# CUAI/Edge-Proposal-Sets

Measured on AMD Instinct MI355X. Metric: candidate edges scored/sec on ogbl-ppa (ppa-like synthetic): Adamic-Adar over the FULL 2-hop non-edge candidate set + top-4M selection, higher is better.
Workload: dtype int64

## Files before the change

### edge-proposal-sets_amd/_lib.py

```python
from __future__ import annotations

import ctypes
import os
import subprocess
import threading

_HERE = os.path.dirname(os.path.abspath(__file__))
LIB_PATH = os.path.join(_HERE, "libeps_hip.so")
CSRC = os.path.join(_HERE, "csrc")

_c = ctypes
_vp, _i64, _i32, _int = _c.c_void_p, _c.c_int64, _c.c_int32, _c.c_int

SIGNATURES = {
    "eps_version": (_int, []),
    "eps_last_error": (_c.c_char_p, []),
    "eps_device_info": (_int, [_c.POINTER(_int), _c.c_char_p, _int]),
    "eps_warm_up": (_int, []),
    "eps_col_sums": (_int, [_vp, _vp, _vp, _i64, _i64, _vp, _vp, _vp]),
    "eps_node_weights": (_int, [_vp, _i64, _int, _vp, _vp]),
    "eps_node_weights_f64": (_int, [_vp, _i64, _int, _vp, _vp]),
    "eps_pair_scores": (_int, [_vp, _vp, _vp, _vp, _i64, _vp, _vp, _i64, _vp, _vp, _vp, _vp]),
    "eps_pair_scores_f64": (_int, [_vp, _vp, _vp, _vp, _i64, _vp, _vp, _i64, _vp, _vp, _vp]),
    "eps_pair_scores_grouped": (_int, [_vp, _vp, _vp, _vp, _i64, _vp, _vp, _i64, _vp, _vp, _vp, _vp]),
# ... 60 lines not shown
    "eps_mlp_decode_bn_stats": (_int, [_vp, _i64, _i32, _vp, _vp, _i64, _c.POINTER(_vp), _c.POINTER(_vp), _i32, _vp, _vp, _vp, _i64, _vp]),
    "eps_mlp_decode_bn_backward": (_int, [_vp, _i64, _i32, _vp, _vp, _i64, _c.POINTER(_vp), _c.POINTER(_vp), _c.POINTER(_vp), _i32,
                                          _c.POINTER(_vp), _c.POINTER(_vp), _vp, _vp, _vp, _c.c_float, _vp, _c.c_float, _vp, _vp, _vp,
                                          _c.POINTER(_vp), _c.POINTER(_vp), _vp, _vp, _vp, _vp, _i64, _vp]),
    "eps_kth_largest_workspace_bytes": (_i64, []),
    "eps_kth_largest_f32": (_int, [_vp, _i64, _i64, _vp, _vp, _vp]),
    "eps_select_topk_rows_relabelled": (_int, [_vp, _vp, _i64, _i64, _i32, _vp, _vp, _vp, _vp, _i64, _vp]),
    "eps_select_topk_rows_pairs": (_int, [_vp, _vp, _i64, _i64, _i32, _vp, _vp, _i64, _vp, _vp, _i64, _vp]),
    "eps_sort_pairs_by_u_workspace_bytes": (_i64, [_i64]),
    "eps_sort_pairs_by_u": (_int, [_vp, _i64, _i32, _i32, _vp, _vp, _i64, _vp]),
    "eps_compact_between": (_int, [_vp, _vp, _i64, _vp, _vp, _vp, _vp, _vp, _vp]),
    "eps_select_compact_workspace_bytes": (_i64, []),
    "eps_select_compact": (_int, [_vp, _vp, _i64, _vp, _i64, _i32, _c.c_float, _c.c_float, _c.c_float, _vp, _vp, _vp, _vp, _i64, _vp, _vp, _vp]),
    "eps_kth_begin": (_int, [_vp, _i64, _vp]),
    "eps_kth_hist_f32": (_int, [_vp, _i64, _vp, _i32, _vp]),
    "eps_kth_pick": (_int, [_vp, _i32, _vp, _vp]),
    "eps_compact_at_least": (_int, [_vp, _vp, _i64, _vp, _vp, _vp, _vp, _vp]),
    "eps_select_topk_cut_workspace_bytes": (_i64, []),
    "eps_compact_survivors": (_int, [_vp, _vp, _i64, _vp, _vp, _vp, _vp, _i64, _vp]),
    "eps_select_topk_cut": (_int, [_vp, _vp, _i64, _i64, _vp, _vp, _vp, _vp, _i64, _vp]),
    "eps_select_topk_rows_workspace_bytes": (_i64, [_i64]),
    "eps_select_topk_rows": (_int, [_vp, _vp, _i64, _i64, _i32, _vp, _vp, _vp, _i64, _vp]),
    "eps_tail_state_bytes": (_i64, []),
    "eps_score_bins": (_i32, []),
    "eps_score_hist_into": (_int, [_vp, _vp, _i64, _vp, _vp, _vp, _vp, _vp]),
    "eps_score_deal_plan": (_int, [_vp, _i64, _i32, _i64, _vp, _vp, _vp, _vp, _vp, _vp]),
    "eps_score_hist": (_int, [_vp, _vp, _i64, _vp, _vp, _vp, _vp, _vp]),
    "eps_score_pick_compact": (_int, [_vp, _vp, _i64, _vp, _vp, _vp, _i64, _i32, _c.c_float, _c.c_float, _c.c_float, _i32, _vp, _vp, _vp,
                                      _vp, _i64, _vp, _vp, _vp]),
    "eps_radix_sort_workspace_bytes": (_i64, [_i64]),
    "eps_radix_sort_by_u": (_int, [_vp, _i64, _vp, _i32, _i32, _vp, _vp, _i64, _vp, _vp]),
    "eps_radix_sort_rows": (_int, [_vp, _vp, _i64, _vp, _i64, _i32, _vp, _vp, _i64, _vp, _vp, _vp, _i64, _vp, _vp]),
    "eps_rescore_runs_dev": (_int, [_vp, _vp, _vp, _i64, _vp, _i64, _vp, _vp, _vp]),
    "eps_pack_keys": (_int, [_vp, _vp, _i64, _i64, _vp, _vp]),
    "eps_unpack_keys": (_int, [_vp, _i64, _vp, _vp, _vp]),
    "eps_two_path_counts": (_int, [_vp, _vp, _i64, _vp, _vp]),
    "eps_katz_workspace_bytes": (_i64, [_i64]),
    "eps_katz_pair_scores": (_int, [_vp, _vp, _vp, _vp, _vp, _vp, _vp, _vp, _i64, _vp, _vp, _i64, _c.c_double, _c.c_double,
                                    _c.c_double, _vp, _vp, _vp]),
    "eps_katz_columns_limits": (_int, [_c.POINTER(_i32), _c.POINTER(_i32)]),
    "eps_katz_columns_workspace_bytes": (_i64, [_i64]),
    "eps_katz_columns_chunk": (_i64, [_i64]),
    "eps_katz_column_scores": (_int, [_vp, _vp, _vp, _vp, _vp, _vp, _vp, _i64, _i64, _i64, _vp, _vp, _i64, _c.c_double, _c.c_double,
                                      _c.c_double, _i64, _i32, _vp, _i64, _vp, _vp]),
    "eps_cos_node_features": (_int, [_vp, _vp, _vp, _i64, _vp, _i64, _i32, _vp, _i64, _vp]),
    "eps_edge_cosines": (_int, [_vp, _vp, _i64, _vp, _i64, _i32, _vp, _vp, _vp]),
    "eps_cos_node_features_nrm": (_int, [_vp, _vp, _vp, _i64, _vp, _i64, _i32, _vp, _i64, _vp, _vp]),
    "eps_pair_cn_backward_workspace_bytes": (_i64, [_i64]),
    "eps_pair_cn_backward": (_int, [_vp, _vp, _vp, _i64, _i64, _vp, _vp, _vp, _i64, _vp, _vp, _i64, _vp]),
    "eps_cos_features_backward": (_int, [_vp, _vp, _vp, _i64, _vp, _i64, _i32, _vp, _vp, _vp, _vp, _vp, _i64, _vp]),
    "eps_csr_merge_workspace_bytes": (_i64, [_i64]),
    "eps_csr_merge_count": (_int, [_vp, _vp, _i64, _vp, _i64, _vp, _vp, _vp, _vp, _i64, _vp]),
    "eps_csr_merge_fill": (_int, [_vp, _vp, _vp, _i64, _vp, _i64, _vp, _vp, _i64, _vp, _vp, _vp]),
    "eps_segment_topk_class_max": (_i64, [_i32]),
    "eps_segment_topk": (_int, [_vp, _vp, _vp, _i64, _i64, _vp, _vp, _vp, _vp]),
    "eps_local_index_pairs": (_int, [_vp, _i64, _vp, _vp, _vp, _i64, _i32, _vp, _vp]),
    "eps_local_index_columns_workspace_bytes": (_i64, [_i64]),
    "eps_local_index_columns": (_int, [_vp, _i64, _i64, _i64, _vp, _vp, _vp, _i64, _vp, _vp, _i32, _vp, _vp, _i64, _vp, _vp, _vp, _vp,
                                       _i64, _vp]),
    "eps_pair_cn_list_limits": (_int, [_c.POINTER(_i32), _c.POINTER(_i32)]),
    "eps_pair_cn_list_count": (_int, [_vp, _vp, _i64, _vp, _vp, _i64, _vp, _vp]),
    "eps_pair_cn_list_fill": (_int, [_vp, _vp, _i64, _vp, _vp, _i64, _vp, _vp, _vp, _vp]),
    "eps_cn_list_transpose_workspace_bytes": (_i64, [_i64, _i64]),
    "eps_cn_list_transpose": (_int, [_vp, _vp, _i64, _i64, _i64, _vp, _vp, _vp, _i64, _vp]),
    "eps_local_community_limits": (_int, [_c.POINTER(_i32), _c.POINTER(_i32), _c.POINTER(_i32)]),
    "eps_local_community_degrees": (_int, [_vp, _vp, _i64, _vp, _vp, _i64, _vp, _vp, _vp]),
# ... 92 lines not shown
```

### edge-proposal-sets_amd/csrc/eps_common.hip

```cpp
#include "eps_common.h"

#include <stdarg.h>
#include <string.h>

#include <atomic>

static thread_local char g_err[512] = "";

void eps_set_error(const char *fmt, ...)
{
    va_list ap;
    va_start(ap, fmt);
    vsnprintf(g_err, sizeof(g_err), fmt, ap);
    va_end(ap);
}

extern "C" const char *eps_last_error(void) { return g_err; }

extern "C" int eps_version(void) { return EPS_ABI_VERSION; }

int eps_num_cus()
{
    static thread_local int cached_dev = -1;
    static thread_local int cached_cus = 256;
// ... 35 lines not shown
    if (hipGetSymbolAddress((void **)counter, HIP_SYMBOL(g_work_counter)) != hipSuccess) {
        eps_set_error("%s: cannot resolve the work counter", who);
        return EPS_ELAUNCH;
    }
    *counter += g_counter_turn.fetch_add(1) % EPS_COUNTER_SLOTS;
    if (hipMemsetAsync(*counter, 0, sizeof(unsigned int), stream) != hipSuccess) {
        eps_set_error("%s: cannot reset the work counter", who);
        return EPS_ELAUNCH;
    }
    return EPS_OK;
}

__device__ unsigned int g_work_counter8[EPS_COUNTER_SLOTS][8];
static std::atomic<unsigned int> g_counter8_turn{0};

int eps_take_counters8(unsigned int **counters, hipStream_t stream, const char *who)
{
    if (hipGetSymbolAddress((void **)counters, HIP_SYMBOL(g_work_counter8)) != hipSuccess) {
        eps_set_error("%s: cannot resolve the work counters", who);
        return EPS_ELAUNCH;
    }
    *counters += 8 * (g_counter8_turn.fetch_add(1) % EPS_COUNTER_SLOTS);
    if (hipMemsetAsync(*counters, 0, 8 * sizeof(unsigned int), stream) != hipSuccess) {
        eps_set_error("%s: cannot reset the work counters", who);
        return EPS_ELAUNCH;
    }
    return EPS_OK;
}

#define EPS_UNITS(X) \
    X(graph_prep) X(csr_merge) X(scan_pieces) X(scan_tables) X(scan_heads) X(rescore) \
    X(pair_intersect) X(pair_grouped) X(expand_score) X(filter_scan) X(spmm_csr) \
    X(gemm_f32) X(dense_cn) X(mlp_decode) X(mlp_decode_bf16) X(mlp_decode_train) X(topk_keys) X(topk_select) X(segment_topk) \
    X(tail_sort) X(katz_pairs) X(katz_columns) X(local_index) X(cosine_cn) X(cosine_cn_bwd) X(pair_cn_list) X(local_community)

#define EPS_DECLARE_WARM(unit) extern "C" void eps_warm_##unit(void *stream);
EPS_UNITS(EPS_DECLARE_WARM)

extern "C" int eps_warm_up(void)
{
    hipStream_t s = nullptr;
    if (hipStreamCreateWithFlags(&s, hipStreamNonBlocking) != hipSuccess) {
        eps_set_error("eps_warm_up: cannot create a stream");
        return EPS_ELAUNCH;
    }
#define EPS_CALL_WARM(unit) eps_warm_##unit(s);
    EPS_UNITS(EPS_CALL_WARM)
    const hipError_t e = hipStreamSynchronize(s);
    (void)hipStreamDestroy(s);
    if (e != hipSuccess) {
        eps_set_error("eps_warm_up: %s", hipGetErrorString(e));
        return EPS_ELAUNCH;
    }
    return EPS_OK;
}
```

### edge-proposal-sets_amd/csrc/tail_sort.hip

```cpp
#include "eps_common.h"
#include <string.h>

#define TS_T 1024
#define TS_W (TS_T / 64)
#define TS_KPT 4
#define TS_TILE (TS_T * TS_KPT)
#define TS_MAXG 256
#define TS_MAXPASS 16

#define TS_MB 8
#define TS_BINS ((32 - TS_MB + 1) << TS_MB)

__device__ __forceinline__ uint32_t ts_ordered(float f)
{
    f = f + 0.0f;
    const uint32_t b = __builtin_bit_cast(uint32_t, f);
    return (b & 0x80000000u) ? ~b : (b | 0x80000000u);
}
__device__ __forceinline__ float ts_unordered(uint32_t o)
{
    const uint32_t b = (o & 0x80000000u) ? (o & 0x7fffffffu) : ~o;
    return __builtin_bit_cast(float, b);
}
__device__ __forceinline__ uint32_t ts_bucket(uint32_t d)
{
    if (d < (1u << TS_MB)) return d;
    const int e = 31 - __clz((int)d);
    return ((uint32_t)(e - TS_MB + 1) << TS_MB) | ((d >> (e - TS_MB)) & ((1u << TS_MB) - 1u));
}
__device__ __forceinline__ uint32_t ts_bucket_floor(uint32_t b)
{
    if (b < (1u << TS_MB)) return b;
    const uint32_t e1 = b >> TS_MB, m = b & ((1u << TS_MB) - 1u);
    return ((1u << TS_MB) | m) << (e1 - 1u);
}

struct ts_sel_state {
    uint32_t hist[TS_BINS];
    uint32_t done;
    uint32_t pad;
    unsigned long long n_out;
};

struct ts_sort_state {
    uint32_t arrive;
    uint32_t leave;
    unsigned long long runs;
    uint32_t totals[TS_MAXPASS][256];
    uint32_t hist[TS_MAXG][256];
};

extern "C" int64_t eps_tail_state_bytes(void)
{
    const size_t a = (sizeof(ts_sel_state) + 255) & ~(size_t)255, b = (sizeof(ts_sort_state) + 255) & ~(size_t)255;
    return (int64_t)(a + b);
}
static ts_sel_state *ts_sel_of(void *state) { return (ts_sel_state *)state; }
static ts_sort_state *ts_sort_of(void *state) { return (ts_sort_state *)((char *)state + ((sizeof(ts_sel_state) + 255) & ~(size_t)255)); }

__global__ __launch_bounds__(TS_T) void ts_hist_kernel(const int64_t *__restrict__ keys, const float *__restrict__ vals, int64_t n_max,
                                                       const unsigned long long *__restrict__ n_dev, const float *__restrict__ base,
                                                       const float *__restrict__ above, uint32_t *__restrict__ hist)
{
    __shared__ uint32_t h[TS_BINS];
    const int tid = threadIdx.x, lane = tid & 63;
    int64_t n = n_max;
    if (n_dev) {
        const unsigned long long c = *n_dev;
// ... 741 lines not shown
```

### edge-proposal-sets_amd/ops.py

```python
from __future__ import annotations

import ctypes
import struct
from typing import Optional, Sequence, Tuple

import torch

from . import _lib

W_AA, W_RA = 0, 1

KERNEL_EVENTS = None
EVENT_NAMES = None
_SCAN_EVENTS = ("scan_piece_kernel", "filter_scan_kernel")

_SCRATCH = {}


def _scratch(name, dev, n_words: int, alloc, zero: bool = False) -> torch.Tensor:
    key = (name, dev.type, dev.index)
    buf = _SCRATCH.get(key)
    if buf is None or buf.numel() < n_words:
        _SCRATCH.pop(key, None)
        buf = None
# ... 1548 lines not shown
        _call("eps_sort_pairs_by_u", dev, keys, n, int(id_bits), int(v_block_shift), out, wsp, wsb, timed=("sort_pairs_by_u", n))
    return out


def _topk_rows(sel_keys, sel_vals, m: int, k: int, id_bits: int, perm, as_pairs: bool = False):
    dev = _need_gpu(sel_keys, sel_vals, perm)
    _chk(_I64, sel_keys=sel_keys, perm=perm); _chk(_F32, sel_vals=sel_vals)
    k = int(k)
    take = min(k, 2 * m)
    rows = torch.empty((2, take) if as_pairs else take, dtype=_I64, device=dev)
    out_v = torch.empty(take, dtype=_F32, device=dev)
    if take:
        _, wsp, wsb = _aligned_ws(dev, _lib.load().eps_select_topk_rows_workspace_bytes(m))
        head = (sel_keys, sel_vals, m, k, int(id_bits))
        if as_pairs:
            _call("eps_select_topk_rows_pairs", dev, *head, perm, rows, take, out_v, wsp, wsb, timed=("select_rows", m))
        elif perm is None:
            _call("eps_select_topk_rows", dev, *head, rows, out_v, wsp, wsb)
        else:
            _call("eps_select_topk_rows_relabelled", dev, *head, perm, rows, out_v, wsp, wsb)
    return rows, out_v


def select_rows(sel_keys: torch.Tensor, sel_vals: torch.Tensor, k: int, id_bits: int = 32,
                perm: Optional[torch.Tensor] = None) -> Tuple[torch.Tensor, torch.Tensor]:
    return _topk_rows(sel_keys, sel_vals, sel_keys.numel(), k, id_bits, perm)


def select_rows_pairs(sel_keys: torch.Tensor, sel_vals: torch.Tensor, k: int, id_bits: int = 32,
                      perm: Optional[torch.Tensor] = None) -> Tuple[torch.Tensor, torch.Tensor]:
    return _topk_rows(sel_keys, sel_vals, sel_keys.numel(), k, id_bits, perm, as_pairs=True)


def select_topk(keys: torch.Tensor, vals: torch.Tensor, k: int, id_bits: int = 32) -> Tuple[torch.Tensor, torch.Tensor]:
    dev = _need_gpu(keys, vals)
    _chk(_I64, keys=keys); _chk(_F32, vals=vals)
    n, k = keys.numel(), int(k)
    if vals.numel() != n:
        raise _lib.EpsError("select_topk: keys and vals differ in length")
    sel_k = torch.empty(n, dtype=_I64, device=dev)
    sel_v = torch.empty(n, dtype=_F32, device=dev)
    n_sel = torch.zeros(1, dtype=_I64, device=dev)
    _, wsp, wsb = _aligned_ws(dev, _lib.load().eps_select_topk_cut_workspace_bytes())
    _call("eps_select_topk_cut", dev, keys, vals, n, k, sel_k, sel_v, n_sel, wsp, wsb)
    return _topk_rows(sel_k, sel_v, int(n_sel.item()), k, id_bits, None)


def tail_state(dev) -> torch.Tensor:
    return _scratch(("tail", torch.cuda.current_stream(dev).cuda_stream), dev, 1,
                    lambda: (int(_lib.load().eps_tail_state_bytes()) + 7) // 8 + 32, zero=True)


def _tail_addr(dev):
    st = tail_state(dev)
    return ctypes.c_void_p(st.data_ptr() + (-st.data_ptr()) % 256)


def tail_state_reset(dev) -> None:
    tail_state(dev).zero_()


def score_hist(keys: Optional[torch.Tensor], vals: torch.Tensor, n_dev, base: torch.Tensor, above: Optional[torch.Tensor] = None) -> None:
    dev = _need_gpu(keys, vals, base, above)
    _chk(_I64, keys=keys, n_dev=n_dev); _chk(_F32, vals=vals, base=base, above=above)
    _call("eps_score_hist", dev, keys, vals, vals.numel(), n_dev, base, above, _tail_addr(dev),
          timed=("select_compact", vals.numel()))
# ... 109 lines not shown
```

### edge-proposal-sets_amd/scan.py

```python
from __future__ import annotations

from collections import namedtuple
from typing import List, Optional, Tuple

import torch

from . import ops
from .graph import CSRGraph

SAMPLE_STRIDE = 256
SAFETY = 2.0
SMALL_SET = 1 << 25
MAX_K = 1 << 30
MAX_LAUNCHES = 8
_CHUNK_SLACK = 8192 * 320
RELABEL_MIN_NODES = 100_000
ONE_PASS = True
_PIECE_SLACK = 8192 * 1024 + 65536
MAX_SCREEN_SHIFT = 30
HEADS = True
HEAD_BETA = 0.5
HEAD_KEEP = (0.3, 0.58)
HEAD_LIST = 2
HEAD_MIN_PATHS = 1 << 30
# ... 578 lines not shown
        bar = torch.where(torch.isinf(vote), -inf, vote)
    return bar


def _gather_varlen(t: torch.Tensor, world: int):
    from . import dist as epd
    n = torch.tensor([t.numel()], dtype=torch.int64, device=t.device)
    lens = torch.cat(epd.all_gather_list(n)).tolist()
    return epd.gather_ragged(t, lens)


def select_topk(keys: torch.Tensor, vals: torch.Tensor, k: int, n_nodes: Optional[int] = None) -> Tuple[torch.Tensor, torch.Tensor]:
    if keys.is_cuda:
        bits = 32 if not n_nodes else max(1, min(32, int(n_nodes - 1).bit_length()))
        return ops.select_topk(keys.contiguous(), vals.contiguous(), k, bits)
    return select_topk_torch(keys, vals, k)


def select_topk_torch(keys: torch.Tensor, vals: torch.Tensor, k: int) -> Tuple[torch.Tensor, torch.Tensor]:
    k2 = (k + 1) // 2
    if vals.numel() > k2:
        kth = torch.sort(vals, descending=True).values[k2 - 1] if k2 >= 1 else float("inf")
        m = vals >= kth
        keys, vals = keys[m], vals[m]
    keys = torch.cat([keys, ((keys & 0xFFFFFFFF) << 32) | (keys >> 32)])
    vals = torch.cat([vals, vals])
    o = torch.argsort(keys)
    keys, vals = keys[o], vals[o]
    o = torch.sort(vals, descending=True, stable=True).indices[:k]
    return keys[o], vals[o]


TAIL_DEVICE = True
TAIL_SORT = "library"
EXACT_SCREENING = True
RESCORE_V_BLOCK = 12
DIST_HIST = True
DIST_ROWS_MIN = 1 << 15


def score_splitters(vals: torch.Tensor, world: int) -> torch.Tensor:
    n = vals.numel()
    samp = torch.sort(vals[::max(1, n // 32768)], descending=True).values
    idx = (torch.arange(1, world, device=vals.device) * samp.numel()) // world
    return samp[idx.clamp(max=samp.numel() - 1)]


def score_range_counts(vals: torch.Tensor, splitters: torch.Tensor) -> torch.Tensor:
    r = (vals.unsqueeze(1) < splitters.unsqueeze(0)).sum(1)
    return torch.bincount(r, minlength=splitters.numel() + 1)


def _ordered_rows_distributed(keys: torch.Tensor, vals: torch.Tensor, k: int, bits: int, perm, rank: int, world: int,
                              rows_on: Optional[int] = None):
    from . import dist as epd
    sp = score_splitters(vals, world)
    counts = score_range_counts(vals, sp).tolist()
    lo = sp[rank:rank + 1] if rank < world - 1 else None
    hi = sp[rank - 1:rank] if rank > 0 else None
    mk, mv, _ = ops.compact_between(keys, vals, lo, hi)
    m = counts[rank]
    rk, rv = ops.select_rows(mk[:m].contiguous(), mv[:m].contiguous(), 2 * m, bits, perm)
    lens = [2 * c for c in counts]
    if rows_on is None:
        rows_k, rows_v = epd.gather_ragged(rk, lens), epd.gather_ragged(rv, lens)
    else:
        rows_k, rows_v = epd.gather_ragged_to(rk, lens, rows_on), epd.gather_ragged_to(rv, lens, rows_on)
# ... 129 lines not shown
                action = "heads off" if head_trouble >= 2 or head_stale >= 3 else "grow walked list" if overflow else "rebuild heads"
                return again(action, "launches with skipped heads", drop_heads)
        slot_overflow = any(t.slots > capacity for t in table)
        if screened and not self.rescore_all and not slot_overflow and any(table[0].cut < t.pre_thr for t in table):
            return again("rescore all", "the re-scoring pre-filter", drop_heads)
        if slot_overflow:
            return Verdict("rescan wider" if table[0].cut_is_neg_inf else "rescan below cut", launches, drop_heads, head_trouble, head_stale)
        n_cand, n_sel = sum(t.candidates for t in table), sum(t.n_sel for t in table)
        if bar_set and n_sel < (k2 if head_budget is not None else min(k2, n_cand)):
            return Verdict("drop bar" if launches > 3 else "lower bar", launches, drop_heads, head_trouble, head_stale)
        return Verdict("done", launches, drop_heads, head_trouble, head_stale)

    def apply(self, v: Verdict, total_half: int, world: int) -> str:
        self.launches, self.head_trouble, self.head_stale = v.launches, v.head_trouble, v.head_stale
        if v.action == "sketch off":
            self.sketch, self.sketch_void = False, self.sketch_void + 1
        elif v.action == "grow walked list":
            self.head_list *= 2
        elif v.action == "heads off":
            self.use_heads = False
        elif v.action == "rescore all":
            self.rescore_all = True
        elif v.action in ("rescan below cut", "rescan wider"):
            self.wanted *= 4
        elif v.action in ("lower bar", "drop bar"):
            self.safety = SAFETY * 8 ** (self.launches - 1)
            self.launches += 1
            if v.action == "drop bar":
                self.wanted = 2 * total_half // world
        return {"rescan below cut": "below cut", "lower bar": "estimate", "drop bar": "none"}.get(v.action, "keep")


def _device_tail(g: CSRGraph, screen: Screen, res: ops.Survivors, bar: torch.Tensor, k: int, k2: int, params, bits: int, perm):
    library = TAIL_SORT == "library"
    room = min(res.capacity, 2 * k2 + (1 << 16))
    while True:
        ops.score_hist(res.key, res.val, res.count_ptr, bar)
        c_keys, c_vals, n_valid, _, pre_thr = ops.score_pick_compact(res.key, res.val, res.count_ptr, bar, k2, mode=2,
                                                                     params=params, room=room, want_vals=screen.exact)
        count, sel_room = n_valid, room
        if library:
            nv = int(n_valid.item())
            if nv > room:
                room = min(res.capacity, nv)
                continue
            c_keys, c_vals = c_keys[:nv], c_vals[:nv] if screen.exact else None
            count, sel_room = None, max(nv, 1)
        if screen.exact:
            x_keys, x_vals = c_keys, c_vals
        elif library:
            x_keys = ops.sort_pairs_by_u(c_keys, bits, RESCORE_V_BLOCK)
            x_vals = ops.rescore_runs(g.rowptr, g.col, screen.fixw, g.n_rows, x_keys)
        else:
            x_keys = ops.radix_sort_by_u(c_keys, n_valid, bits, RESCORE_V_BLOCK)
            x_vals = ops.rescore_runs_dev(g.rowptr, g.col, screen.fixw, g.n_rows, x_keys, n_valid)
        ops.score_hist(x_keys, x_vals, count, bar, above=bar)
        sel_k, sel_v, n_sel, cut, _ = ops.score_pick_compact(x_keys, x_vals, count, bar, k2, above=bar, swap_halves=not screen.exact,
                                                             room=sel_room)
        row = (res.rec[1:2], res.rec[4:5], n_sel, cut, res.status, pre_thr, res.walked_slots, bar)
        if library:
            return [_unpack_status(_pack_status(*row).tolist())], sel_k, sel_v, cut, 0 if screen.exact else nv, None
        r_pairs, r_scores, n_rows = ops.radix_sort_rows(sel_k, sel_v, n_sel, k, bits, perm)
        st, (nv, n_out) = _unpack_status(_pack_status(*row, extra=(n_valid, n_rows)).tolist(), extra=2)
        if nv <= room:
            return [st], sel_k, sel_v, cut, 0 if screen.exact else nv, (r_pairs, r_scores, n_out)
        room = min(res.capacity, nv)


def _prefilter(g: CSRGraph, screen: Screen, res: ops.Survivors, bar, k2: int, params, world: int, rescore_all: bool):
    k_pre = 0 if rescore_all else (k2 + world - 1) // world
    room = res.capacity if rescore_all else min(res.capacity, 2 * k_pre + (1 << 16))
    c_keys, c_vals, n_valid, _, pre_thr = ops.select_compact(res.key, res.val, k_pre, res.count_ptr, mode=2, params=params, room=room)
    nv = int(n_valid.item())
    if nv > room:
        c_keys, c_vals, n_valid, _, pre_thr = ops.select_compact(res.key, res.val, k_pre, res.count_ptr, mode=2, params=params,
                                                                 room=min(res.capacity, nv))
        nv = int(n_valid.item())
    if screen.exact:
        return c_keys[:nv], c_vals[:nv], pre_thr, 0, room
    keys, vals = rescore_exact(g, screen, c_keys[:nv], bar)
    return keys, vals, pre_thr, nv, room


def _read_exchange(got: torch.Tensor, nsel_all: torch.Tensor, cut: torch.Tensor, counts: torch.Tensor, world: int):
    rows = got[:, :_STATUS_WORDS].reshape(-1).to(torch.int64)
    flat = torch.cat([rows, cut.view(torch.int32).to(torch.int64), nsel_all, counts.reshape(-1)]).tolist()
    nsel, deal = flat[rows.numel() + 1:][:world], flat[rows.numel() + 1 + world:]
    return ([_unpack_status(flat[r * _STATUS_WORDS:(r + 1) * _STATUS_WORDS])._replace(n_sel=nsel[r], cut_bits=flat[rows.numel()])
             for r in range(world)], [deal[r * world:(r + 1) * world] for r in range(world)])


def _cut_from_histograms(keys: torch.Tensor, vals: torch.Tensor, row, k2: int, bar: torch.Tensor, world: int):
    from . import dist as epd
    bins = ops.score_bins()
    send = torch.zeros(_XCHG_HEAD + bins, dtype=torch.int32, device=vals.device)
    send[:_STATUS_WORDS] = _pack_status(**row)
    ops.score_hist_into(keys, vals, None, bar, send[_XCHG_HEAD:], above=bar)
    got = epd._gather_into(send, world).view(world, _XCHG_HEAD + bins)
# ... 97 lines not shown
    g, perm = scan_graph(g0, relabel)
    fixw = _scan_weights(g0, g, perm, node_w) if g.val is None else None
    mine = shard_columns(g, rank, world)
    total_half = total_half_paths(g)
    k2 = (k + 1) // 2
    bits = max(1, min(32, int(g.n_rows - 1).bit_length()))
    screen = screen_weights(g0, g, perm, node_w) if one_pass_available(g) else None
    if screen is not None and not screen.usable:
        screen = None
    if screen is None and g.val is not None:
        raise ops._lib.EpsError("scan_topk: this weighted graph / weight table does not fit the one-pass scan (see scan_available)")
    slack = _CHUNK_SLACK if screen is None else _PIECE_SLACK
    sampled = total_half > SMALL_SET and SAFETY * k < total_half
    bar = estimate_bar(g, fixw, k, rank=rank, world=world, screen=screen) if sampled else None
    state = _Retry(int(sampled), (2 * total_half if bar is None else int(2 * SAFETY * k)) // world, HEAD_LIST, sketch=SKETCH_PIECES,
                   use_heads=bool(HEADS and screen is not None and screen.has_plan and screen.ssum is not None and g.val is None
                                  and total_half >= HEAD_MIN_PATHS))
    capacity = _capacity(state.wanted, slack)
    _count_scan(g, screen)
    n_rescored = None
    while True:
        if state.launches >= MAX_LAUNCHES:
            raise ops._lib.EpsError(f"scan_topk: no usable bar after {state.launches} launches (k = {k}, capacity {capacity})")
        def sketch_for(budget):
            return bool(state.sketch and screen is not None and screen_variant(g) == 2 and not screen.exact
                        and (int(screen.w_max_units) + 2) * SKETCH_PIECE_PATHS < 1 << 32
                        and budget >= HEAD_BETA * SKETCH_MIN_PATHS * screen.w_max_units)
        ht = (_heads_for(g, screen, bar, sketch_for) if state.use_heads and bar is not None else None)
        walked_cap = max(1, min(int(state.head_list * capacity), ops.SURVIVOR_SLOTS_MAX)) if ht is not None else 0
        res = _launch(g, fixw, mine if ht is None else live_columns(g, screen, ht, rank, world), float("-inf") if bar is None else bar,
                      capacity, both=True, screen=screen, heads=ht, walked_capacity=walked_cap, sketch=ht is not None and sketch_for(ht.budget))
        state.launches += 1
        rows = deal = None
        if screen is not None:
            params = screen.lower_params(max_degree(g), None if ht is None else ht.d_used) + (4e-6,)
        if (TAIL_DEVICE and not _sharded(world) and screen is not None and g.val is None and bar is not None and not state.rescore_all
                and k2 + (1 << 16) < (1 << 30)):
            table, sel_k, sel_v, cut, n_rescored, rows = _device_tail(g, screen, res, bar, k, k2, params, bits, perm)
        else:
            keys, vals, pre_thr, room = res.key, res.val, None, 0
            if screen is not None:
                keys, vals, pre_thr, n_rescored, room = _prefilter(g, screen, res, bar, k2, params, world, state.rescore_all)
            row = dict(slots=res.rec[1:2], candidates=res.rec[4:5], status=None if screen is None else res.status, pre_thr=pre_thr,
                       walked=res.walked_slots, bar=bar)
            exchange = _sharded(world) and screen is not None and not state.rescore_all
            sel_k, sel_v, cut, table, deal = (_cut_from_histograms(keys, vals, row, k2, bar, world) if exchange and bar is not None and DIST_HIST
                                              else _cut_from_scores(keys, vals, row, k2, room, world) if exchange
                                              else _cut_local(keys, vals, row, k2, screen is not None, world))
        v = state.verdict(table, capacity=capacity, walked_cap=walked_cap, head_budget=None if ht is None else ht.budget,
                          shift=None if ht is None else screen.shift, screened=screen is not None, k2=k2, bar_set=bar is not None)
        new_bar = state.apply(v, total_half, world)
        if v.drop_heads:
            screen.head_cur = None
        if v.action == "done":
            break
        if new_bar == "below cut":
            bar = torch.nextafter(cut, torch.full_like(cut, float("-inf")))
        elif new_bar == "estimate":
            bar = estimate_bar(g, fixw, k, safety=state.safety, rank=rank, world=world, screen=screen)
            if bar is None:
                state.wanted = 2 * total_half // world
        elif new_bar == "none":
            bar = None
        capacity = _capacity(state.wanted, slack)
    if screen is not None and bar is not None and 0.0 < table[0].bar < float("inf"):
        screen.bar_hint[(k, sample_stride(k), float(SAFETY))] = table[0].bar
    pairs, scores, shard = ((rows[0][:, :rows[2]], rows[1][:rows[2]], None) if rows is not None else
                            _ordered_rows(sel_k, sel_v, [t.n_sel for t in table], deal, k, bits, perm, rank, world, rows_on))
    if stats is not None:
        _step_stats(stats, g, screen, fixw, table, ht, capacity, state, n_rescored, shard, bar, rank, world)
    return pairs, scores
```

### include/eps_abi.h

```cpp
#ifndef EPS_ABI_H
#define EPS_ABI_H

#include <stdint.h>

#ifdef __cplusplus
extern "C" {
#endif

#define EPS_ABI_VERSION 7

#define EPS_OK 0
#define EPS_EINVAL (-1)
#define EPS_ELAUNCH (-2)
#define EPS_ENODEV (-3)

#define EPS_W_AA 0
#define EPS_W_RA 1

int eps_version(void);
const char *eps_last_error(void);

int eps_warm_up(void);

int eps_device_info(int *n_cu, char *name, int name_len);
// ... 224 lines not shown
int64_t eps_sort_pairs_by_u_workspace_bytes(int64_t n);
int eps_sort_pairs_by_u(const int64_t *keys, int64_t n, int32_t id_bits, int32_t v_block_shift, int64_t *out_by_u, void *workspace,
                        int64_t workspace_bytes, void *stream);
int64_t eps_select_topk_cut_workspace_bytes(void);
int eps_compact_survivors(const int64_t *keys, const float *vals, int64_t n, int64_t *out_keys, float *out_vals,
                          int64_t *n_out, void *workspace, int64_t workspace_bytes, void *stream);
int eps_compact_at_least(const int64_t *keys, const float *vals, int64_t n, const float *cut_or_null, int64_t *out_keys,
                         float *out_vals, int64_t *n_out, void *stream);
int eps_select_topk_cut(const int64_t *keys, const float *vals, int64_t n, int64_t k, int64_t *sel_keys, float *sel_vals,
                        int64_t *n_sel, void *workspace, int64_t workspace_bytes, void *stream);
int64_t eps_select_topk_rows_workspace_bytes(int64_t m);
int eps_select_topk_rows(const int64_t *sel_keys, const float *sel_vals, int64_t m, int64_t k, int32_t id_bits,
                         int64_t *out_keys, float *out_vals, void *workspace, int64_t workspace_bytes, void *stream);
int64_t eps_tail_state_bytes(void);
int32_t eps_score_bins(void);
int eps_score_hist_into(const int64_t *keys_or_null, const float *vals, int64_t n_max, const unsigned long long *n_dev_or_null,
                        const float *base, const float *above_or_null, uint32_t *hist, void *stream);
int eps_score_deal_plan(const uint32_t *hists, int64_t row_stride, int32_t world, int64_t k, const float *base, float *cut,
                        float *splitters, int64_t *counts, int64_t *nsel, void *stream);
int eps_score_hist(const int64_t *keys_or_null, const float *vals, int64_t n_max, const unsigned long long *n_dev_or_null,
                   const float *base, const float *above_or_null, void *state, void *stream);
int eps_score_pick_compact(const int64_t *keys_or_null, const float *vals, int64_t n_max, const unsigned long long *n_dev_or_null,
                           const float *base, const float *above_or_null, int64_t k, int32_t mode, float pa, float pb, float pc,
                           int32_t swap_halves, float *kth_or_null, float *thr_or_null, int64_t *out_keys_or_null,
                           float *out_vals_or_null, int64_t out_cap, int64_t *n_out_or_null, void *state, void *stream);
int64_t eps_radix_sort_workspace_bytes(int64_t n_records);
int eps_radix_sort_by_u(const int64_t *keys, int64_t n_max, const int64_t *n_dev_or_null, int32_t id_bits, int32_t v_block_shift,
                        int64_t *out_by_u, void *workspace, int64_t workspace_bytes, void *state, void *stream);
int eps_radix_sort_rows(const int64_t *sel_keys, const float *sel_vals, int64_t m_max, const int64_t *m_dev_or_null, int64_t k,
                        int32_t id_bits, const int64_t *perm_or_null, int64_t *out_pairs, int64_t out_ld, float *out_scores,
                        int64_t *n_rows_out_or_null, void *workspace, int64_t workspace_bytes, void *state, void *stream);
int eps_rescore_runs_dev(const int64_t *rowptr, const int32_t *col, const int64_t *fixw, int64_t n_nodes, const int64_t *keys,
                         int64_t n_max, const int64_t *n_dev, float *out, void *stream);
int eps_pack_keys(const float *score, const int64_t *ids_or_null, int64_t id_base, int64_t n,
                  int64_t *keys, void *stream);
int eps_unpack_keys(const int64_t *keys, int64_t n, float *score_or_null, int64_t *id_or_null,
                    void *stream);

int eps_two_path_counts(const int64_t *rowptr, const int32_t *col, int64_t n_nodes, int64_t *paths, void *stream);
int64_t eps_katz_workspace_bytes(int64_t n_pairs);
int eps_katz_pair_scores(const int64_t *rowptr, const int32_t *col, const float *val, const int64_t *rowptr_t,
                         const int32_t *col_t, const float *val_t, const int64_t *paths_out, const int64_t *paths_in,
                         int64_t n_nodes, const int32_t *u, const int32_t *v, int64_t n_pairs, double c1, double c2,
                         double c3, void *workspace, float *out, void *stream);

int eps_katz_columns_limits(int32_t *lds_capacity, int32_t *chunk);
int64_t eps_katz_columns_chunk(int64_t n_cand);
int64_t eps_katz_columns_workspace_bytes(int64_t max_support);
int eps_katz_column_scores(const int64_t *rowptr, const int32_t *col, const float *val, const int64_t *rowptr_t,
                           const int32_t *col_t, const float *val_t, const int64_t *paths_in, int64_t n_nodes,
                           int64_t v_lo, int64_t v_hi, const int64_t *colptr, const int32_t *cand_u, int64_t n_cand,
                           double c1, double c2, double c3, int64_t max_support, int32_t chunk, void *workspace,
                           int64_t workspace_bytes, float *out, void *stream);

int eps_cos_node_features(const int64_t *rowptr, const int32_t *col, const float *val, int64_t n_rows,
                          const float *x, int64_t ldx, int32_t f, float *xhat, int64_t ldh, void *stream);
int eps_edge_cosines(const int64_t *rowptr, const int32_t *col, int64_t n_rows, const float *xhat, int64_t ldh,
                     int32_t f, const int32_t *revpos, float *c, void *stream);

int eps_cos_node_features_nrm(const int64_t *rowptr, const int32_t *col, const float *val, int64_t n_rows,
                              const float *x, int64_t ldx, int32_t f, float *xhat, int64_t ldh, float *nrm, void *stream);
int64_t eps_pair_cn_backward_workspace_bytes(int64_t nnz);
int eps_pair_cn_backward(const int64_t *rowptr, const int32_t *col, const float *c, int64_t n_rows, int64_t nnz,
                         const int32_t *u, const int32_t *v, const float *g, int64_t n_pairs, float *gc, void *workspace,
                         int64_t workspace_bytes, void *stream);
int eps_cos_features_backward(const int64_t *rowptr, const int32_t *col, const float *val, int64_t n_rows,
// ... 44 lines not shown
```

Measured before the change: 1321 billion.

## Build top-k output rows by sorting all rescored pairs by score in one pass

Adds a device tail path that radix-sorts all rescored pairs by score in descending order, with swapped-halves keys as the tie-break. One block then finds the live count and the bucketed cut, and a windowed expand kernel writes both directed rows of each pair in rank order, resolving ties within equal-score runs. The default tail mode becomes this path whenever screening is inexact. It replaces the histogram, pick-compact and separate row-sort sequence with one full sort of n records, which may cost more than the old path when n is much larger than k2. If a tie run exceeds the window, the kernel sets a flag and the output falls back to the library path.

```diff
diff --git a/edge-proposal-sets_amd/_lib.py b/edge-proposal-sets_amd/_lib.py
--- a/edge-proposal-sets_amd/_lib.py
+++ b/edge-proposal-sets_amd/_lib.py
@@ -116,6 +116,10 @@
     "eps_radix_sort_by_u": (_int, [_vp, _i64, _vp, _i32, _i32, _vp, _vp, _i64, _vp, _vp]),
     "eps_radix_sort_rows": (_int, [_vp, _vp, _i64, _vp, _i64, _i32, _vp, _vp, _i64, _vp, _vp, _vp, _i64, _vp, _vp]),
     "eps_rescore_runs_dev": (_int, [_vp, _vp, _vp, _i64, _vp, _i64, _vp, _vp, _vp]),
+    "eps_rows_by_score_max_run": (_i32, []),
+    "eps_rows_by_score_window": (_i32, []),
+    "eps_rows_by_score_workspace_bytes": (_i64, [_i64]),
+    "eps_rows_by_score": (_int, [_vp, _vp, _i64, _vp, _i64, _i64, _i32, _vp, _vp, _vp, _vp, _vp, _vp, _vp, _i64, _vp, _vp, _i64, _vp]),
     "eps_pack_keys": (_int, [_vp, _vp, _i64, _i64, _vp, _vp]),
     "eps_unpack_keys": (_int, [_vp, _i64, _vp, _vp, _vp]),
     "eps_two_path_counts": (_int, [_vp, _vp, _i64, _vp, _vp]),
diff --git a/edge-proposal-sets_amd/csrc/eps_common.hip b/edge-proposal-sets_amd/csrc/eps_common.hip
--- a/edge-proposal-sets_amd/csrc/eps_common.hip
+++ b/edge-proposal-sets_amd/csrc/eps_common.hip
@@ -91,7 +91,7 @@
     X(graph_prep) X(csr_merge) X(scan_pieces) X(scan_tables) X(scan_heads) X(rescore) \
     X(pair_intersect) X(pair_grouped) X(expand_score) X(filter_scan) X(spmm_csr) \
     X(gemm_f32) X(dense_cn) X(mlp_decode) X(mlp_decode_bf16) X(mlp_decode_train) X(topk_keys) X(topk_select) X(segment_topk) \
-    X(tail_sort) X(katz_pairs) X(katz_columns) X(local_index) X(cosine_cn) X(cosine_cn_bwd) X(pair_cn_list) X(local_community)
+    X(tail_sort) X(rows_by_score) X(katz_pairs) X(katz_columns) X(local_index) X(cosine_cn) X(cosine_cn_bwd) X(pair_cn_list) X(local_community)
 
 #define EPS_DECLARE_WARM(unit) extern "C" void eps_warm_##unit(void *stream);
 EPS_UNITS(EPS_DECLARE_WARM)
diff --git a/edge-proposal-sets_amd/csrc/rows_by_score.hip b/edge-proposal-sets_amd/csrc/rows_by_score.hip
--- /dev/null
+++ b/edge-proposal-sets_amd/csrc/rows_by_score.hip
@@ -0,0 +1,167 @@
+#include "eps_common.h"
+#include "score_buckets.h"
+
+#include <rocprim/device/device_radix_sort.hpp>
+#include <rocprim/iterator/transform_iterator.hpp>
+
+#define RBS_T 1024
+#define RBS_L 1024
+
+struct rbs_swap_halves {
+    __host__ __device__ int64_t operator()(int64_t k) const { return (int64_t)(((uint64_t)k << 32) | ((uint64_t)k >> 32)); }
+};
+using rbs_keys_in = rocprim::transform_iterator<const int64_t *, rbs_swap_halves, int64_t>;
+
+template <class Pred>
+__device__ int64_t rbs_prefix_len(const float *__restrict__ s, int64_t n, Pred pred)
+{
+    int64_t lo = 0, hi = n;
+    while (lo < hi) {
+        const int64_t step = (hi - lo + RBS_T - 1) / RBS_T, idx = lo + (int64_t)threadIdx.x * step;
+        const int c = __syncthreads_count(idx < hi && pred(s[idx]));
+        if (c == 0) {
+            hi = lo;
+        } else {
+            const int64_t last = lo + (int64_t)(c - 1) * step;
+            lo = last + 1;
+            hi = last + step < hi ? last + step : hi;
+        }
+    }
+    return lo;
+}
+
+__global__ __launch_bounds__(RBS_T) void rbs_cut_kernel(const float *__restrict__ s, int64_t n, const float *__restrict__ bar, uint64_t k2,
+                                                        float *__restrict__ cut_out, int64_t *__restrict__ n_sel_out,
+                                                        int64_t *__restrict__ flag)
+{
+    const float floor_v = *bar;
+    const int64_t n_live = rbs_prefix_len(s, n, [=](float x) { return x > floor_v && x > -__builtin_inff(); });
+    float cut = -__builtin_inff();
+    int64_t n_sel = n_live;
+    if (k2 != 0 && (uint64_t)n_live >= k2) {
+        const uint32_t ob = ts_ordered(floor_v), o = ts_ordered(s[k2 - 1]);
+        const uint32_t b = ts_bucket(o > ob ? o - ob : 0u);
+        if (b != 0u) {
+            const uint64_t e = (uint64_t)ob + ts_bucket_floor(b);
+            cut = ts_unordered(e > 0xFFFFFFFFull ? 0xFFFFFFFFu : (uint32_t)e);
+            n_sel = rbs_prefix_len(s, n_live, [=](float x) { return x >= cut; });
+        }
+    }
+    if (threadIdx.x == 0) {
+        *cut_out = cut;
+        *n_sel_out = n_sel;
+        *flag = 0;
+    }
+}
+
+__global__ __launch_bounds__(RBS_T) void rbs_expand_kernel(const int64_t *__restrict__ sk, const float *__restrict__ sv,
+                                                           const int64_t *__restrict__ n_sel_p, const int64_t *__restrict__ perm, int64_t k,
+                                                           int64_t *__restrict__ out_pairs, int64_t ld, float *__restrict__ out_vals,
+                                                           int64_t *__restrict__ flag)
+{
+    __shared__ uint64_t lk[RBS_T + RBS_L];
+    __shared__ float ls[RBS_T + RBS_L];
+    const int64_t n_sel = *n_sel_p;
+    const int64_t w0 = (int64_t)blockIdx.x * RBS_T;
+    if (w0 >= n_sel) return;
+    const int tid = threadIdx.x;
+    const int64_t w1 = w0 + RBS_T < n_sel ? w0 + RBS_T : n_sel;
+    auto fetch = [&](int64_t j, int slot, float x) {
+        const uint64_t key = (uint64_t)sk[j];
+        uint64_t a = key & 0xFFFFFFFFull, b = key >> 32;
+        if (perm) {
+            a = (uint64_t)perm[a];
+            b = (uint64_t)perm[b];
+        }
+        lk[slot] = a < b ? (a << 32) | b : (b << 32) | a;
+        ls[slot] = x;
+    };
+    if (w0 + tid < w1) fetch(w0 + tid, tid, sv[w0 + tid]);
+    bool reach = false;
+    if (w1 == w0 + RBS_T && w1 + tid < n_sel) {
+        const float x = sv[w1 + tid];
+        reach = x == sv[w1 - 1];
+        if (reach) fetch(w1 + tid, RBS_T + tid, x);
+    }
+    const int n_reach = __syncthreads_count(reach), lim = (int)(w1 - w0) + n_reach;
+    auto place = [&](int p) {
+        const float mine = ls[p];
+        int s = p;
+        while (s > 0 && ls[s - 1] == mine) --s;
+        if (s == 0 && w0 > 0 && sv[w0 - 1] == mine) return;
+        int e = p + 1;
+        while (e < lim && ls[e] == mine) ++e;
+        if (e - s > RBS_L) {
+            *flag = 1;
+            return;
+        }
+        const uint64_t kb = lk[p], ka = (kb << 32) | (kb >> 32);
+        int ra = 0, rb = 0;
+        for (int q = s; q < e; ++q) {
+            const uint64_t cb = lk[q], ca = (cb << 32) | (cb >> 32);
+            ra += (int)(ca < ka) + (int)(cb < ka);
+            rb += (int)(ca < kb) + (int)(cb < kb);
+        }
+        const int64_t row0 = 2 * (w0 + s), row_a = row0 + ra, row_b = row0 + rb;
+        if (row_a < k) {
+            out_pairs[row_a] = (int64_t)(kb >> 32);
+            out_pairs[ld + row_a] = (int64_t)(kb & 0xFFFFFFFFull);
+            out_vals[row_a] = mine;
+        }
+        if (row_b < k) {
+            out_pairs[row_b] = (int64_t)(kb & 0xFFFFFFFFull);
+            out_pairs[ld + row_b] = (int64_t)(kb >> 32);
+            out_vals[row_b] = mine;
+        }
+    };
+    if (w0 + tid < w1) place(tid);
+    if (tid < n_reach) place(RBS_T + tid);
+}
+
+static size_t rbs_sort_temp_bytes(int64_t n)
+{
+    size_t b = 0;
+    (void)rocprim::radix_sort_pairs_desc((void *)nullptr, b, (const float *)nullptr, (float *)nullptr, rbs_keys_in(nullptr, rbs_swap_halves()),
+                                         (int64_t *)nullptr, (size_t)n, 0u, 32u, (hipStream_t)0);
+    return b;
+}
+
+extern "C" int32_t eps_rows_by_score_max_run(void) { return RBS_L; }
+extern "C" int32_t eps_rows_by_score_window(void) { return RBS_T; }
+
+extern "C" int64_t eps_rows_by_score_workspace_bytes(int64_t n)
+{
+    if (n <= 0) return 256;
+    return (int64_t)((rbs_sort_temp_bytes(n) + 255) & ~(size_t)255);
+}
+
+extern "C" int eps_rows_by_score(const int64_t *keys_by_u, const float *vals, int64_t n, const float *bar, int64_t k2, int64_t k,
+                                 int32_t id_bits, const int64_t *perm_or_null, int64_t *sorted_keys, float *sorted_vals, float *cut,
+                                 int64_t *n_sel, int64_t *flag, int64_t *out_pairs, int64_t pairs_ld, float *out_vals, void *workspace,
+                                 int64_t workspace_bytes, void *stream)
+{
+    EPS_REQUIRE(n >= 0 && n < (1ll << 31) && k2 >= 0 && k >= 0 && id_bits >= 1 && id_bits <= 32, "eps_rows_by_score: bad argument");
+    EPS_REQUIRE(bar && cut && n_sel && flag, "eps_rows_by_score: null pointer");
+    hipStream_t s = (hipStream_t)stream;
+    if (n != 0) {
+        EPS_REQUIRE(keys_by_u && vals && sorted_keys && sorted_vals, "eps_rows_by_score: null pointer");
+        EPS_REQUIRE(k == 0 || (out_pairs && out_vals && pairs_ld >= (k < 2 * n ? k : 2 * n)), "eps_rows_by_score: out_pairs / pairs_ld too small");
+        EPS_REQUIRE(workspace && ((uintptr_t)workspace & 255) == 0 && workspace_bytes >= eps_rows_by_score_workspace_bytes(n),
+                    "eps_rows_by_score: needs a 256-byte aligned workspace of eps_rows_by_score_workspace_bytes(n) bytes");
+        size_t temp_bytes = (size_t)workspace_bytes;
+        if (rocprim::radix_sort_pairs_desc(workspace, temp_bytes, vals, sorted_vals, rbs_keys_in(keys_by_u, rbs_swap_halves()), sorted_keys,
+                                           (size_t)n, 0u, 32u, s) != hipSuccess) {
+            eps_set_error("eps_rows_by_score: radix sort failed");
+            return EPS_ELAUNCH;
+        }
+    }
+    hipLaunchKernelGGL(rbs_cut_kernel, dim3(1), dim3(RBS_T), 0, s, sorted_vals, n, bar, (uint64_t)k2, cut, n_sel, flag);
+    if (n != 0 && k != 0)
+        hipLaunchKernelGGL(rbs_expand_kernel, dim3((unsigned)((n + RBS_T - 1) / RBS_T)), dim3(RBS_T), 0, s, sorted_keys, sorted_vals, n_sel,
+                           perm_or_null, k, out_pairs, pairs_ld, out_vals, flag);
+    EPS_CHECK_LAUNCH("eps_rows_by_score");
+    return EPS_OK;
+}
+
+__global__ void rows_by_score_warm_kernel() {}
+extern "C" void eps_warm_rows_by_score(void *stream) { hipLaunchKernelGGL(rows_by_score_warm_kernel, dim3(1), dim3(1), 0, (hipStream_t)stream); }
diff --git a/edge-proposal-sets_amd/csrc/score_buckets.h b/edge-proposal-sets_amd/csrc/score_buckets.h
--- /dev/null
+++ b/edge-proposal-sets_amd/csrc/score_buckets.h
@@ -0,0 +1,29 @@
+#pragma once
+#include <stdint.h>
+
+#define TS_MB 8
+#define TS_BINS ((32 - TS_MB + 1) << TS_MB)
+
+__device__ __forceinline__ uint32_t ts_ordered(float f)
+{
+    f = f + 0.0f;
+    const uint32_t b = __builtin_bit_cast(uint32_t, f);
+    return (b & 0x80000000u) ? ~b : (b | 0x80000000u);
+}
+__device__ __forceinline__ float ts_unordered(uint32_t o)
+{
+    const uint32_t b = (o & 0x80000000u) ? (o & 0x7fffffffu) : ~o;
+    return __builtin_bit_cast(float, b);
+}
+__device__ __forceinline__ uint32_t ts_bucket(uint32_t d)
+{
+    if (d < (1u << TS_MB)) return d;
+    const int e = 31 - __clz((int)d);
+    return ((uint32_t)(e - TS_MB + 1) << TS_MB) | ((d >> (e - TS_MB)) & ((1u << TS_MB) - 1u));
+}
+__device__ __forceinline__ uint32_t ts_bucket_floor(uint32_t b)
+{
+    if (b < (1u << TS_MB)) return b;
+    const uint32_t e1 = b >> TS_MB, m = b & ((1u << TS_MB) - 1u);
+    return ((1u << TS_MB) | m) << (e1 - 1u);
+}
diff --git a/edge-proposal-sets_amd/csrc/tail_sort.hip b/edge-proposal-sets_amd/csrc/tail_sort.hip
--- a/edge-proposal-sets_amd/csrc/tail_sort.hip
+++ b/edge-proposal-sets_amd/csrc/tail_sort.hip
@@ -1,4 +1,5 @@
 #include "eps_common.h"
+#include "score_buckets.h"
 #include <string.h>
 
 #define TS_T 1024
@@ -8,32 +9,6 @@
 #define TS_MAXG 256
 #define TS_MAXPASS 16
 
-#define TS_MB 8
-#define TS_BINS ((32 - TS_MB + 1) << TS_MB)
-
-__device__ __forceinline__ uint32_t ts_ordered(float f)
-{
-    f = f + 0.0f;
-    const uint32_t b = __builtin_bit_cast(uint32_t, f);
-    return (b & 0x80000000u) ? ~b : (b | 0x80000000u);
-}
-__device__ __forceinline__ float ts_unordered(uint32_t o)
-{
-    const uint32_t b = (o & 0x80000000u) ? (o & 0x7fffffffu) : ~o;
-    return __builtin_bit_cast(float, b);
-}
-__device__ __forceinline__ uint32_t ts_bucket(uint32_t d)
-{
-    if (d < (1u << TS_MB)) return d;
-    const int e = 31 - __clz((int)d);
-    return ((uint32_t)(e - TS_MB + 1) << TS_MB) | ((d >> (e - TS_MB)) & ((1u << TS_MB) - 1u));
-}
-__device__ __forceinline__ uint32_t ts_bucket_floor(uint32_t b)
-{
-    if (b < (1u << TS_MB)) return b;
-    const uint32_t e1 = b >> TS_MB, m = b & ((1u << TS_MB) - 1u);
-    return ((1u << TS_MB) | m) << (e1 - 1u);
-}
 
 struct ts_sel_state {
     uint32_t hist[TS_BINS];
diff --git a/edge-proposal-sets_amd/ops.py b/edge-proposal-sets_amd/ops.py
--- a/edge-proposal-sets_amd/ops.py
+++ b/edge-proposal-sets_amd/ops.py
@@ -1604,6 +1604,30 @@
     return _topk_rows(sel_keys, sel_vals, sel_keys.numel(), k, id_bits, perm, as_pairs=True)
 
 
+def rows_by_score_limits() -> Tuple[int, int]:
+    lib = _lib.load()
+    return int(lib.eps_rows_by_score_max_run()), int(lib.eps_rows_by_score_window())
+
+
+def rows_by_score(keys_by_u: torch.Tensor, vals: torch.Tensor, bar: torch.Tensor, k2: int, k: int, id_bits: int = 32,
+                  perm: Optional[torch.Tensor] = None):
+    dev = _need_gpu(keys_by_u, vals, bar, perm)
+    _chk(_I64, keys_by_u=keys_by_u, perm=perm); _chk(_F32, vals=vals, bar=bar)
+    n, k = keys_by_u.numel(), int(k)
+    _chk_len("rows_by_score", "vals", vals, n, "one score per pair")
+    cap = min(k, 2 * n)
+    pairs = torch.empty((2, cap), dtype=_I64, device=dev)
+    scores = torch.empty(cap, dtype=_F32, device=dev)
+    sorted_k = torch.empty(n, dtype=_I64, device=dev)
+    sorted_v = torch.empty(n, dtype=_F32, device=dev)
+    cut = torch.empty(1, dtype=_F32, device=dev)
+    words = torch.empty(2, dtype=_I64, device=dev)
+    _, wsp, wsb = _aligned_ws(dev, _lib.load().eps_rows_by_score_workspace_bytes(n))
+    _call("eps_rows_by_score", dev, keys_by_u, vals, n, bar, int(k2), k, int(id_bits), perm, sorted_k, sorted_v, cut, words.data_ptr(),
+          words.data_ptr() + 8, pairs, cap, scores, wsp, wsb, timed=("select_rows", n))
+    return pairs, scores, sorted_k, sorted_v, words[0:1], cut, words[1:2]
+
+
 def select_topk(keys: torch.Tensor, vals: torch.Tensor, k: int, id_bits: int = 32) -> Tuple[torch.Tensor, torch.Tensor]:
     dev = _need_gpu(keys, vals)
     _chk(_I64, keys=keys); _chk(_F32, vals=vals)
diff --git a/edge-proposal-sets_amd/scan.py b/edge-proposal-sets_amd/scan.py
--- a/edge-proposal-sets_amd/scan.py
+++ b/edge-proposal-sets_amd/scan.py
@@ -634,7 +634,7 @@
 
 
 TAIL_DEVICE = True
-TAIL_SORT = "library"
+TAIL_SORT = "score"
 EXACT_SCREENING = True
 RESCORE_V_BLOCK = 12
 DIST_HIST = True
@@ -830,7 +830,8 @@
 
 
 def _device_tail(g: CSRGraph, screen: Screen, res: ops.Survivors, bar: torch.Tensor, k: int, k2: int, params, bits: int, perm):
-    library = TAIL_SORT == "library"
+    library = TAIL_SORT != "radix"
+    by_score = TAIL_SORT == "score" and not screen.exact
     room = min(res.capacity, 2 * k2 + (1 << 16))
     while True:
         ops.score_hist(res.key, res.val, res.count_ptr, bar)
@@ -852,16 +853,23 @@
         else:
             x_keys = ops.radix_sort_by_u(c_keys, n_valid, bits, RESCORE_V_BLOCK)
             x_vals = ops.rescore_runs_dev(g.rowptr, g.col, screen.fixw, g.n_rows, x_keys, n_valid)
+        if by_score:
+            r_pairs, r_scores, sel_k, sel_v, n_sel, cut, flag = ops.rows_by_score(x_keys, x_vals, bar, k2, k, bits, perm)
+            row = (res.rec[1:2], res.rec[4:5], n_sel, cut, res.status, pre_thr, res.walked_slots, bar)
+            st, (void,) = _unpack_status(_pack_status(*row, extra=(flag,)).tolist(), extra=1)
+            rows = None if void else (r_pairs, r_scores, min(k, 2 * st.n_sel))
+            return [st], sel_k, sel_v, cut, nv, rows, "library" if void else "score"
         ops.score_hist(x_keys, x_vals, count, bar, above=bar)
         sel_k, sel_v, n_sel, cut, _ = ops.score_pick_compact(x_keys, x_vals, count, bar, k2, above=bar, swap_halves=not screen.exact,
                                                              room=sel_room)
         row = (res.rec[1:2], res.rec[4:5], n_sel, cut, res.status, pre_thr, res.walked_slots, bar)
         if library:
-            return [_unpack_status(_pack_status(*row).tolist())], sel_k, sel_v, cut, 0 if screen.exact else nv, None
+            return ([_unpack_status(_pack_status(*row).tolist())], sel_k, sel_v, cut, 0 if screen.exact else nv, None,
+                    "library")
         r_pairs, r_scores, n_rows = ops.radix_sort_rows(sel_k, sel_v, n_sel, k, bits, perm)
         st, (nv, n_out) = _unpack_status(_pack_status(*row, extra=(n_valid, n_rows)).tolist(), extra=2)
         if nv <= room:
-            return [st], sel_k, sel_v, cut, 0 if screen.exact else nv, (r_pairs, r_scores, n_out)
+            return [st], sel_k, sel_v, cut, 0 if screen.exact else nv, (r_pairs, r_scores, n_out), "radix"
         room = min(res.capacity, nv)
 
 
@@ -1025,11 +1033,12 @@
                       capacity, both=True, screen=screen, heads=ht, walked_capacity=walked_cap, sketch=ht is not None and sketch_for(ht.budget))
         state.launches += 1
         rows = deal = None
+        rows_path = "library"
         if screen is not None:
             params = screen.lower_params(max_degree(g), None if ht is None else ht.d_used) + (4e-6,)
         if (TAIL_DEVICE and not _sharded(world) and screen is not None and g.val is None and bar is not None and not state.rescore_all
                 and k2 + (1 << 16) < (1 << 30)):
-            table, sel_k, sel_v, cut, n_rescored, rows = _device_tail(g, screen, res, bar, k, k2, params, bits, perm)
+            table, sel_k, sel_v, cut, n_rescored, rows, rows_path = _device_tail(g, screen, res, bar, k, k2, params, bits, perm)
         else:
             keys, vals, pre_thr, room = res.key, res.val, None, 0
             if screen is not None:
@@ -1062,4 +1071,5 @@
                             _ordered_rows(sel_k, sel_v, [t.n_sel for t in table], deal, k, bits, perm, rank, world, rows_on))
     if stats is not None:
         _step_stats(stats, g, screen, fixw, table, ht, capacity, state, n_rescored, shard, bar, rank, world)
+        stats["rows_path"] = rows_path
     return pairs, scores
diff --git a/include/eps_abi.h b/include/eps_abi.h
--- a/include/eps_abi.h
+++ b/include/eps_abi.h
@@ -280,6 +280,12 @@
                         int64_t *n_rows_out_or_null, void *workspace, int64_t workspace_bytes, void *state, void *stream);
 int eps_rescore_runs_dev(const int64_t *rowptr, const int32_t *col, const int64_t *fixw, int64_t n_nodes, const int64_t *keys,
                          int64_t n_max, const int64_t *n_dev, float *out, void *stream);
+int32_t eps_rows_by_score_max_run(void);
+int32_t eps_rows_by_score_window(void);
+int64_t eps_rows_by_score_workspace_bytes(int64_t n);
+int eps_rows_by_score(const int64_t *keys_by_u, const float *vals, int64_t n, const float *bar, int64_t k2, int64_t k, int32_t id_bits,
+                      const int64_t *perm_or_null, int64_t *sorted_keys, float *sorted_vals, float *cut, int64_t *n_sel, int64_t *flag,
+                      int64_t *out_pairs, int64_t pairs_ld, float *out_vals, void *workspace, int64_t workspace_bytes, void *stream);
 int eps_pack_keys(const float *score, const int64_t *ids_or_null, int64_t id_base, int64_t n,
                   int64_t *keys, void *stream);
 int eps_unpack_keys(const int64_t *keys, int64_t n, float *score_or_null, int64_t *id_or_null,
```

Measured after the change: 1366 billion (median of 6 runs). +3.4%, better.
